# eukaryo/smith-waterman-simd

Measured on AMD Instinct MI355X. Metric: alignments/sec (and GCUPS) on 1M fixed-length pairs, 1/2/4/8 MI355X, higher is better.
Workload: dtype u16

## Files before the change

### smith-waterman-simd_amd/csrc/sw_kernels.hip

```cpp
#include "swmi_internal.h"

#include <type_traits>
#include <utility>

namespace swmi {
namespace {

constexpr int kSeqLen = 128;
constexpr int kWavesPerBlock = 4;


__device__ __forceinline__ int max_i16(int a, int b)
{
    const short r = __builtin_elementwise_max((short)a, (short)b);
    return (int)(unsigned short)r;
}

template <bool I16>
__device__ __forceinline__ int vmax(int a, int b)
{
    if constexpr (I16) return max_i16(a, b);
    else return a > b ? a : b;
}

template <bool I16>
__device__ __forceinline__ int sat_sub(int a, int b)
{
    if constexpr (I16) return (int)(unsigned short)__builtin_elementwise_sub_sat((unsigned short)a, (unsigned short)b);
    else return (int)__builtin_elementwise_sub_sat((unsigned)a, (unsigned)b);
}

__device__ __forceinline__ int keep(int v)
{
    asm volatile("" : "+v"(v));
    return v;
}

template <int L>
__device__ __forceinline__ int from_prev_lane(int v, int group_mask)
{
    if constexpr (L == 64) {
#ifdef SWMI_AB_SHFL_UP
        const int s = __shfl_up(v, 1);
        return (threadIdx.x & 63) ? s : 0;
#else
        return __builtin_amdgcn_update_dpp(0, v, 0x138 , 0xf, 0xf, true);
#endif
    } else if constexpr (L == 32) {
        return __builtin_amdgcn_update_dpp(0, v, 0x138, 0xf, 0xf, true) & group_mask;
    } else if constexpr (L == 16) {
        return __builtin_amdgcn_update_dpp(0, v, 0x111 , 0xf, 0xf, true);
    } else {
        return __builtin_amdgcn_update_dpp(0, v, 0x111, 0xf, 0xf, true) & group_mask;
    }
}

template <int R>
__device__ __forceinline__ void load_bases(const uint8_t *p, uint32_t (&w)[(R + 3) / 4])
{
    if constexpr (R == 2) {
        w[0] = *reinterpret_cast<const uint16_t *>(p);
    } else if constexpr (R == 4) {
        w[0] = *reinterpret_cast<const uint32_t *>(p);
    } else if constexpr (R == 8) {
        const uint2 v = *reinterpret_cast<const uint2 *>(p);
        w[0] = v.x; w[1] = v.y;
    } else {
#pragma unroll
        for (int k = 0; k < R / 16; ++k) {
            const uint4 v = *reinterpret_cast<const uint4 *>(p + 16 * k);
            w[4 * k + 0] = v.x; w[4 * k + 1] = v.y; w[4 * k + 2] = v.z; w[4 * k + 3] = v.w;
        }
    }
}

__device__ __forceinline__ uint32_t spread4(uint32_t v)
{
    return (v | (v << 6) | (v << 12) | (v << 18)) & 0x03030303u;
}

template <int R>
__device__ __forceinline__ void load_bases_packed(const uint8_t *p, uint32_t (&w)[(R + 3) / 4])
{
    if constexpr (R == 2) {
        w[0] = 0;
    } else if constexpr (R == 4) {
        w[0] = spread4(p[0]);
    } else if constexpr (R == 8) {
        const uint32_t v = *reinterpret_cast<const uint16_t *>(p);
        w[0] = spread4(v & 0xff); w[1] = spread4(v >> 8);
    } else if constexpr (R == 16) {
        const uint32_t v = *reinterpret_cast<const uint32_t *>(p);
#pragma unroll
        for (int k = 0; k < 4; ++k) w[k] = spread4((v >> (8 * k)) & 0xff);
    } else {
#pragma unroll
        for (int q = 0; q < R / 32; ++q) {
            const uint2 v = *reinterpret_cast<const uint2 *>(p + 8 * q);
#pragma unroll
            for (int k = 0; k < 4; ++k) {
                w[8 * q + k] = spread4((v.x >> (8 * k)) & 0xff);
                w[8 * q + 4 + k] = spread4((v.y >> (8 * k)) & 0xff);
            }
        }
    }
}

template <int L, bool FOLD, bool I16, int MODE>
__global__ void __launch_bounds__(64 * kWavesPerBlock)
sw128_kernel(const uint8_t *__restrict__ seq1s, const uint8_t *__restrict__ seq2s, int32_t *__restrict__ scores,
             uint32_t n, SmRows rows, int gap)
{
    constexpr int R = kSeqLen / L;
    constexpr int A = 64 / L;
    constexpr int PAD = L + 2;
    constexpr int S = kSeqLen + 2 * PAD;
    constexpr int T2 = (kSeqLen + L) / 2;
    constexpr int NW = (R + 3) / 4;

    constexpr bool kWideProfile = true;
    using profile_t = std::conditional_t<kWideProfile, uint32_t, uint16_t>;
    __shared__ profile_t lds_profile[kWavesPerBlock][A * S];
    __shared__ uint32_t lds_rows[kWavesPerBlock][4];
#ifndef SWMI_LDS_BEST_NUM
#define SWMI_LDS_BEST_NUM (R >= 64 ? 0 : R >= 32 ? 1 : R >= 16 ? 2 : R >= 8 ? 1 : 0)
#define SWMI_LDS_BEST_DEN (R >= 64 ? 1 : R >= 32 ? 2 : R >= 16 ? 3 : R >= 8 ? 2 : 1)
#endif
    constexpr int kBestNum = I16 ? 0 : SWMI_LDS_BEST_NUM, kBestDen = SWMI_LDS_BEST_DEN;
    __shared__ int lds_best[kWavesPerBlock][64];
    lds_best[threadIdx.x >> 6][threadIdx.x & 63] = 0;

    const int lane = threadIdx.x & 63;
    const int wv = threadIdx.x >> 6;
    const int g = lane / L;
    const int j = lane % L;
    const uint32_t first_pair = (blockIdx.x * kWavesPerBlock + wv) * A;
    if (first_pair >= n) return;
    uint32_t pair = first_pair + g;
    const bool live = pair < n;
    if (!live) pair = n - 1;

    uint32_t a_w[NW], b_w[NW];
    if constexpr (MODE == 1) {
        if constexpr (R == 2) {
            const uint32_t sh = 4 * (j & 1);
            a_w[0] = spread4((seq1s[(size_t)pair * 32 + (j >> 1)] >> sh) & 0xf);
            b_w[0] = spread4((seq2s[(size_t)pair * 32 + (j >> 1)] >> sh) & 0xf);
        } else {
            load_bases_packed<R>(seq1s + (size_t)pair * 32 + j * (R / 4), a_w);
            load_bases_packed<R>(seq2s + (size_t)pair * 32 + j * (R / 4), b_w);
        }
    } else {
        load_bases<R>(seq1s + (size_t)pair * kSeqLen + j * R, a_w);
        load_bases<R>(seq2s + (MODE == 2 ? (size_t)0 : (size_t)pair * kSeqLen) + j * R, b_w);
    }

    if (lane < 4) lds_rows[wv][lane] = rows.r[lane];
    profile_t *prof = &lds_profile[wv][g * S];
    for (int k = j; k < PAD; k += L) {
        prof[k] = 0;
        prof[PAD + kSeqLen + k] = 0;
    }
#pragma unroll
    for (int i = 0; i < R; ++i) {
        const uint32_t b = (b_w[i / 4] >> (8 * (i % 4))) & 3u;
        prof[PAD + j * R + i] = kWideProfile ? (profile_t)(1u << (8u * b)) : (profile_t)(0x100u | (8u * b));
    }
    __builtin_amdgcn_fence(__ATOMIC_RELEASE, "wavefront");
    __builtin_amdgcn_wave_barrier();
    __builtin_amdgcn_fence(__ATOMIC_ACQUIRE, "wavefront");

    int row_scores[R];
#pragma unroll
    for (int i = 0; i < R; ++i) {
        const uint32_t a = (a_w[i / 4] >> (8 * (i % 4))) & 3u;
        row_scores[i] = (int)lds_rows[wv][a];
    }

    __builtin_amdgcn_s_setprio(2);

    constexpr bool kKeepG = !FOLD && !I16;
    int h[R];
    int hg[kKeepG ? R : 1];
#pragma unroll
    for (int i = 0; i < R; ++i) h[i] = 0;
#pragma unroll
    for (int i = 0; i < (kKeepG ? R : 1); ++i) hg[i] = 0;
    int best = 0;
    int u0 = 0, u1 = 0;
    const int group_mask = keep(j == 0 ? 0 : -1);
    const profile_t *col = prof + PAD - j;

    auto step = [&](uint32_t entry, int up, int diag) {
        const int onehot = kWideProfile ? (int)entry : (int)((entry >> 8) << (entry & 31u));
        int dprev = diag;
        if constexpr (kKeepG) up = sat_sub<false>(up, gap);
#pragma unroll
        for (int i = 0; i < R; ++i) {
            const int left = h[i];
            const int tsum = __builtin_amdgcn_sdot4(row_scores[i], onehot, dprev, true);
            int hn;
            if constexpr (FOLD) {
                const int lu = left > up ? left : up;
                const int x = lu > tsum ? lu : tsum;
                if constexpr (I16) best = keep(max_i16(best, x));
                else if (i % kBestDen < kBestNum) __hip_atomic_fetch_max(&lds_best[wv][lane], x, __ATOMIC_RELAXED, __HIP_MEMORY_SCOPE_WAVEFRONT);
                else best = vmax<false>(best, x);
                hn = sat_sub<I16>(x, gap);
                up = hn;
            } else if constexpr (I16) {
                const int m = keep(max_i16(left, up));
                hn = keep(max_i16(sat_sub<true>(m, gap), tsum));
                best = keep(max_i16(best, hn));
                up = hn;
            } else {
                const int gl = hg[i];
                const int lu = gl > up ? gl : up;
                hn = lu > tsum ? lu : tsum;
                if (i % kBestDen < kBestNum) __hip_atomic_fetch_max(&lds_best[wv][lane], hn, __ATOMIC_RELAXED, __HIP_MEMORY_SCOPE_WAVEFRONT);
                else best = vmax<false>(best, hn);
                const int gn = sat_sub<false>(hn, gap);
                hg[i] = gn;
                up = gn;
            }
            h[i] = hn;
            dprev = left;
        }
        return from_prev_lane<L>(h[R - 1], group_mask);
    };

    uint32_t e0 = col[0];
    for (int t2 = 0; t2 < T2; ++t2) {
        const uint32_t e1 = col[2 * t2 + 1];
        const uint32_t e2 = col[2 * t2 + 2];
        u1 = step(e0, u0, u1);
        u0 = step(e1, u1, u0);
        e0 = e2;
    }

    if constexpr (kBestNum > 0) {
        const int from_lds = lds_best[wv][lane];
        best = best > from_lds ? best : from_lds;
    }
#pragma unroll
    for (int o = L / 2; o > 0; o >>= 1) {
        const int other = __shfl_xor(best, o);
        best = best > other ? best : other;
    }
    if constexpr (FOLD) best = best > gap ? best - gap : 0;
    if (j == 0 && live) scores[pair] = best;
}


__device__ __forceinline__ uint32_t pk_max3(uint32_t a, uint32_t b, uint32_t c)
{
    uint32_t r;
    asm("v_pk_maximum3_f16 %0, %1, %2, %3" : "=v"(r) : "v"(a), "v"(b), "v"(c));
    return r;
}
__device__ __forceinline__ void keep_f16_denormals()
{
    asm volatile("s_setreg_imm32_b32 hwreg(HW_REG_MODE, 6, 2), 3");
}

constexpr uint32_t kPkLimit = 0x7C00u;
constexpr uint32_t kBPerThread = 1024;
__global__ void __launch_bounds__(256)
pk_max3_selftest_kernel(unsigned long long *__restrict__ counts )
{
    keep_f16_denormals();
    const uint32_t a = blockIdx.x * 256 + threadIdx.x;
    const uint32_t b0 = blockIdx.y * kBPerThread;
    if (a >= kPkLimit) return;
    auto imax3 = [](uint32_t p, uint32_t q, uint32_t r) { const uint32_t m = p > q ? p : q; return m > r ? m : r; };
    auto pk_max3 = [](uint32_t p, uint32_t q, uint32_t r) {
        uint32_t o;
        asm volatile("v_pk_maximum3_f16 %0, %1, %2, %3\n\ts_nop 1" : "=v"(o) : "v"(p), "v"(q), "v"(r));
        return o;
    };
    uint32_t bad = 0, done = 0;
    for (uint32_t b = b0; b < b0 + kBPerThread && b < kPkLimit; ++b) {
        uint32_t h = (a * 0x9E3779B1u) ^ (b * 0x85EBCA77u);
        h ^= h >> 15; h *= 0x2C1B3C6Du; h ^= h >> 12;
        const uint32_t r = h % kPkLimit, r2 = (h >> 7) % kPkLimit;
        const uint32_t x = a | (b << 16), y = b | (r << 16), z = r2 | (a << 16);
        bad += pk_max3(x, y, z) != (imax3(a, b, r2) | (imax3(b, r, a) << 16));
        bad += pk_max3(z, x, y) != (imax3(r2, a, b) | (imax3(a, b, r) << 16));
        bad += pk_max3(y, z, x) != (imax3(b, r2, a) | (imax3(r, a, b) << 16));
        bad += pk_max3(x, y, x) != (imax3(a, b, a) | (imax3(b, r, b) << 16));
        bad += pk_max3(x, y, y) != (imax3(a, b, b) | (imax3(b, r, r) << 16));
        bad += pk_max3(x, x, y) != (imax3(a, a, b) | (imax3(b, b, r) << 16));
        done += 6;
    }
    atomicAdd(&counts[0], (unsigned long long)done);
    if (bad) atomicAdd(&counts[1], (unsigned long long)bad);
}
template <bool LAST>
__device__ __forceinline__ void pk_two_rows(uint32_t &hq0, uint32_t &hq1, uint32_t &hu0, uint32_t &hu1, uint32_t &best, uint32_t &t,
                                            uint32_t &sc, uint32_t up, uint32_t sel2, uint32_t sel3, uint32_t cx, uint32_t cy,
                                            uint32_t gq2, uint32_t q2)
{
    uint32_t x0, x1, s2;
    if constexpr (!LAST) {
        asm volatile("v_pk_maximum3_f16 %[x0], %[hq0], %[up], %[t]\n\t"
                     "v_add_u32 %[t], %[hu0], %[sc]\n\t"
                     "s_nop 0\n\t"
                     "v_pk_sub_u16 %[hu0], %[x0], %[gq] clamp\n\t"
                     "v_perm_b32 %[s2], %[cy], %[cx], %[sel2]\n\t"
                     "v_add_u32 %[hq0], %[q], %[hu0]\n\t"
                     "s_nop 0\n\t"
                     "v_pk_maximum3_f16 %[x1], %[hq1], %[hq0], %[t]\n\t"
                     "v_add_u32 %[t], %[hu1], %[s2]\n\t"
                     "s_nop 0\n\t"
                     "v_pk_sub_u16 %[hu1], %[x1], %[gq] clamp\n\t"
                     "v_perm_b32 %[sc], %[cy], %[cx], %[sel3]\n\t"
                     "s_nop 0\n\t"
                     "v_add_u32 %[hq1], %[q], %[hu1]\n\t"
                     "v_pk_maximum3_f16 %[best], %[best], %[x0], %[x1]"
                     : [hq0] "+v"(hq0), [hq1] "+v"(hq1), [hu0] "+v"(hu0), [hu1] "+v"(hu1), [best] "+v"(best), [t] "+v"(t),
                       [sc] "+v"(sc), [x0] "=&v"(x0), [x1] "=&v"(x1), [s2] "=&v"(s2)
                     : [up] "v"(up), [sel2] "v"(sel2), [sel3] "v"(sel3), [cx] "v"(cx), [cy] "v"(cy), [gq] "s"(gq2), [q] "s"(q2));
    } else {
        asm volatile("v_pk_maximum3_f16 %[x0], %[hq0], %[up], %[t]\n\t"
                     "v_add_u32 %[t], %[hu0], %[sc]\n\t"
                     "s_nop 0\n\t"
                     "v_pk_sub_u16 %[hu0], %[x0], %[gq] clamp\n\t"
                     "s_nop 0\n\t"
                     "v_add_u32 %[hq0], %[q], %[hu0]\n\t"
                     "s_nop 0\n\t"
                     "v_pk_maximum3_f16 %[x1], %[hq1], %[hq0], %[t]\n\t"
                     "s_nop 0\n\t"
                     "v_pk_sub_u16 %[hu1], %[x1], %[gq] clamp\n\t"
                     "v_pk_maximum3_f16 %[best], %[best], %[x0], %[x1]\n\t"
                     "v_add_u32 %[hq1], %[q], %[hu1]"
                     : [hq0] "+v"(hq0), [hq1] "+v"(hq1), [hu0] "+v"(hu0), [hu1] "+v"(hu1), [best] "+v"(best), [t] "+v"(t),
                       [x0] "=&v"(x0), [x1] "=&v"(x1)
                     : [up] "v"(up), [sc] "v"(sc), [gq] "s"(gq2), [q] "s"(q2));
    }
}

enum PkVariant : int { kPkQ0 = 0, kPkBias = 1, kPkVert = 2 };
constexpr int kPkProductBit = 1 << 16;

template <int MODE, int VARIANT, int L>
__global__ void __launch_bounds__(64 * kWavesPerBlock) __attribute__((amdgpu_waves_per_eu(4)))
sw128_pk_kernel(const uint8_t *__restrict__ seq1s, const uint8_t *__restrict__ seq2s, int32_t *__restrict__ scores,
                uint32_t n, SmRows rows ,
                int gap, int q_arg )
{
    const int q = VARIANT == kPkVert ? q_arg & (kPkProductBit - 1) : q_arg;
    const bool product = VARIANT == kPkVert && (q_arg & kPkProductBit) != 0;
    static_assert(L == 4 || L == 8 || L == 16, "lanes per pair of alignments");
    constexpr bool kGenerated = VARIANT == kPkQ0 || VARIANT == kPkVert;
    constexpr int R = kSeqLen / L;
    constexpr int G = 64 / L;
    constexpr int A = 2 * G;
    constexpr int PAD = L + 2;
    constexpr int S = kSeqLen + 2 * PAD;
    constexpr int T2 = (kSeqLen + L - 1) / 2;
    constexpr int NW = R / 4;
    constexpr uint32_t kPadCode = 16u | (16u << 16);
    const bool flag_form = VARIANT == kPkVert && q != 0;

    __shared__ uint32_t lds_col[kWavesPerBlock][G * S];
    __shared__ uint32_t lds_tab[8];

    const int lane = threadIdx.x & 63;
    const int wv = threadIdx.x >> 6;
    const int g = lane / L, j = lane % L;
    const uint32_t first = (blockIdx.x * kWavesPerBlock + wv) * A;
    if (first >= n) return;
    uint32_t px = first + 2 * g, py = px + 1;
    const bool live_x = px < n, live_y = py < n;
    if (!live_x) px = n - 1;
    if (!live_y) py = n - 1;

    uint32_t ax[NW], bx[NW], ay[NW], by[NW];
    if constexpr (MODE == 1) {
        load_bases_packed<R>(seq1s + (size_t)px * 32 + j * (R / 4), ax);
        load_bases_packed<R>(seq2s + (size_t)px * 32 + j * (R / 4), bx);
        load_bases_packed<R>(seq1s + (size_t)py * 32 + j * (R / 4), ay);
        load_bases_packed<R>(seq2s + (size_t)py * 32 + j * (R / 4), by);
    } else {
        load_bases<R>(seq1s + (size_t)px * kSeqLen + j * R, ax);
        load_bases<R>(seq2s + (MODE == 2 ? (size_t)0 : (size_t)px * kSeqLen) + j * R, bx);
        load_bases<R>(seq1s + (size_t)py * kSeqLen + j * R, ay);
        load_bases<R>(seq2s + (MODE == 2 ? (size_t)0 : (size_t)py * kSeqLen) + j * R, by);
    }

    if (lane < 5) {
        uint32_t c = flag_form ? 0x80808080u : 0u;
        if (lane < 4) {
            c = 0;
#pragma unroll
            for (int a = 0; a < 4; ++a) c |= ((rows.r[a] >> (8 * lane)) & 0xFFu) << (8 * a);
        }
        lds_tab[lane] = c;
    }
    uint32_t *prof = &lds_col[wv][g * S];
    const uint32_t pad_code = product ? 0u : kPadCode;
    for (int k = j; k < PAD; k += L) {
        prof[k] = pad_code;
        prof[PAD + kSeqLen + k] = pad_code;
    }
    const uint32_t sel_shift = flag_form ? 8u : 0u, sel_const = flag_form ? 0x000D000Du : 0x0C000C00u;
    uint32_t rsel[R];
    if (product) {
#pragma unroll
        for (int w = 0; w < NW; ++w) {
            const uint32_t cx4 = bx[w] & 0x03030303u, cy4 = by[w] & 0x03030303u;
            const uint32_t ra4 = ax[w] & 0x03030303u, rb4 = ay[w] & 0x03030303u;
#pragma unroll
            for (int k = 0; k < 4; ++k) {
                const uint32_t pick = (uint32_t)k | 0x0C000C00u | ((uint32_t)(4 + k) << 16);
                const uint32_t ce = __builtin_amdgcn_perm(cy4, cx4, pick), re = __builtin_amdgcn_perm(rb4, ra4, pick);
                prof[PAD + j * R + 4 * w + k] = __builtin_amdgcn_perm(rows.r[3], rows.r[2], ((ce * 0x101u) << 1) + 0x01000100u);
                rsel[4 * w + k] = __builtin_amdgcn_perm(rows.r[1], rows.r[0], ((re * 0x101u) << 1) + 0x01000100u);
            }
        }
    } else {
#pragma unroll
    for (int w = 0; w < NW; ++w) {
        const uint32_t cx4 = (bx[w] & 0x03030303u) << 2, cy4 = (by[w] & 0x03030303u) << 2;
        const uint32_t ra4 = ax[w] & 0x03030303u, rb4 = (ay[w] & 0x03030303u) | 0x04040404u;
#pragma unroll
        for (int k = 0; k < 4; ++k) {
            const uint32_t pick = (uint32_t)k | 0x0C000C00u | ((uint32_t)(4 + k) << 16);
            prof[PAD + j * R + 4 * w + k] = __builtin_amdgcn_perm(cy4, cx4, pick);
            if constexpr (VARIANT == kPkVert) rsel[4 * w + k] = (__builtin_amdgcn_perm(rb4, ra4, pick) << sel_shift) | sel_const;
            else                              rsel[4 * w + k] = __builtin_amdgcn_perm(rb4, ra4, pick) | 0x0C000C00u;
        }
    }
    }
    __builtin_amdgcn_fence(__ATOMIC_RELEASE, "wavefront");
    __builtin_amdgcn_wave_barrier();
    __builtin_amdgcn_fence(__ATOMIC_ACQUIRE, "wavefront");
    __builtin_amdgcn_s_setprio(2);

    keep_f16_denormals();

    const uint32_t gq2 = (uint32_t)(gap + q) | ((uint32_t)(gap + q) << 16);
    const uint32_t q2 = (uint32_t)q | ((uint32_t)q << 16);
    uint32_t best = 0;
    const int group_mask = keep(j == 0 ? 0 : -1);
    const uint32_t *col = prof + PAD - j;
    auto tables = [&](uint32_t code, uint32_t &cx, uint32_t &cy) {
        cx = *reinterpret_cast<const uint32_t *>(reinterpret_cast<const char *>(lds_tab) + (code & 0xFFFFu));
        cy = *reinterpret_cast<const uint32_t *>(reinterpret_cast<const char *>(lds_tab) + (code >> 16));
    };
    auto tables_at = [&](int t, uint32_t &cx, uint32_t &cy) {
        const uint16_t *half = reinterpret_cast<const uint16_t *>(col + t);
        cx = *reinterpret_cast<const uint32_t *>(reinterpret_cast<const char *>(lds_tab) + half[0]);
        cy = *reinterpret_cast<const uint32_t *>(reinterpret_cast<const char *>(lds_tab) + half[1]);
    };

    if constexpr (kGenerated) {
#define pk_best best
#define pk_dval(r) ((uint32_t)(gap * ((r) + 1)) * 0x10001u)
        if constexpr (VARIANT == kPkQ0 && R == 32) {
#define PK_SECTION 32
#include "pk_sweeps_gen.inc"
#undef PK_SECTION
        } else if constexpr (VARIANT == kPkQ0 && R == 16) {
#define PK_SECTION 16
#include "pk_sweeps_gen.inc"
#undef PK_SECTION
        } else if constexpr (VARIANT == kPkQ0 && R == 8) {
#define PK_SECTION 8
#include "pk_sweeps_gen.inc"
#undef PK_SECTION
        } else if (product) {
            if constexpr (R == 32) {
#define PK_SECTION 432
#include "pk_sweeps_gen.inc"
#undef PK_SECTION
            } else if constexpr (R == 16) {
#define PK_SECTION 416
#include "pk_sweeps_gen.inc"
#undef PK_SECTION
            } else {
#define PK_SECTION 408
#include "pk_sweeps_gen.inc"
#undef PK_SECTION
            }
        } else if (flag_form) {
            if constexpr (R == 32) {
#define PK_SECTION 332
#include "pk_sweeps_gen.inc"
#undef PK_SECTION
            } else if constexpr (R == 16) {
#define PK_SECTION 316
#include "pk_sweeps_gen.inc"
#undef PK_SECTION
            } else {
#define PK_SECTION 308
#include "pk_sweeps_gen.inc"
#undef PK_SECTION
            }
        } else if constexpr (VARIANT == kPkVert && R == 32) {
#define PK_SECTION 232
#include "pk_sweeps_gen.inc"
#undef PK_SECTION
        } else if constexpr (VARIANT == kPkVert && R == 16) {
#define PK_SECTION 216
#include "pk_sweeps_gen.inc"
#undef PK_SECTION
        } else {
#define PK_SECTION 208
#include "pk_sweeps_gen.inc"
#undef PK_SECTION
        }
#undef pk_best
#undef pk_dval
    } else {
    uint32_t hq[R], hu_[R];
#pragma unroll
    for (int i = 0; i < R; ++i) { hq[i] = q2; hu_[i] = 0; }
    uint32_t u0 = q2, u1 = q2;
    const uint32_t edge = (uint32_t)keep((int)(j == 0 ? q2 : 0u));

    auto step = [&](uint32_t cx, uint32_t cy, uint32_t up, uint32_t diag) {
        const uint32_t d0 = diag - q2;
        uint32_t t = d0 + __builtin_amdgcn_perm(cy, cx, rsel[0]);
        uint32_t sc = __builtin_amdgcn_perm(cy, cx, rsel[1]);
#pragma unroll
        for (int i = 0; i < R; i += 2) {
            if (i + 2 < R) pk_two_rows<false>(hq[i], hq[i + 1], hu_[i], hu_[i + 1], best, t, sc, up, rsel[i + 2], rsel[i + 3], cx, cy, gq2, q2);
            else           pk_two_rows<true>(hq[i], hq[i + 1], hu_[i], hu_[i + 1], best, t, sc, up, 0, 0, cx, cy, gq2, q2);
            up = hq[i + 1];
        }
        asm volatile("s_nop 1");
        uint32_t out = (uint32_t)from_prev_lane<L>((int)hq[R - 1], group_mask);
        return out | edge;
    };
    uint32_t c1 = col[1], x0, y0;
    tables(col[0], x0, y0);
    for (int t2 = 0; t2 < T2; ++t2) {
        const uint32_t c2 = col[2 * t2 + 2], c3 = col[2 * t2 + 3];
        uint32_t x1, y1, x2, y2;
        tables(c1, x1, y1);
        u1 = step(x0, y0, u0, u1);
        tables(c2, x2, y2);
        u0 = step(x1, y1, u1, u0);
        x0 = x2; y0 = y2; c1 = c3;
    }
    step(x0, y0, u0, u1);
    }

#pragma unroll
    for (int o = L / 2; o > 0; o >>= 1) {
        const uint32_t other = (uint32_t)__shfl_xor((int)best, o);
        best = pk_max3(best, other, other);
    }
    const int bx_score = (int)(best & 0xFFFFu), by_score = (int)(best >> 16), gq = VARIANT != kPkVert ? gap + q : flag_form ? gap : 0;
    int sx = bx_score > gq ? bx_score - gq : 0, sy = by_score > gq ? by_score - gq : 0;
    if (flag_form) {
        sx = sx * q / 255;
        sy = sy * q / 255;
    }
    if (j == 0) {
        if (live_x) scores[px] = sx;
        if (live_y) scores[py] = sy;
    }
}

template <int ROW>
__device__ __forceinline__ void fetch_score(int &dst, uint32_t lds_addr)
{
    asm volatile("ds_read_i8 %0, %1 offset:%2" : "=v"(dst) : "v"(lds_addr), "i"(ROW * 256));
}
template <int R, int... I>
__device__ __forceinline__ void fetch_scores_impl(int (&dst)[R], uint32_t lds_addr, std::integer_sequence<int, I...>)
{
    (fetch_score<I>(dst[I], lds_addr), ...);
}
template <int R>
__device__ __forceinline__ void fetch_scores(int (&dst)[R], uint32_t lds_addr)
{
    fetch_scores_impl<R>(dst, lds_addr, std::make_integer_sequence<int, R>{});
}
template <int R>
__device__ __forceinline__ void land_scores(int (&s)[R])
{
    asm volatile("s_waitcnt lgkmcnt(0)" ::: "memory");
#pragma unroll
    for (int i = 0; i < R; ++i) asm volatile("" : "+v"(s[i]));
}

template <int L, int MODE>
__global__ void __launch_bounds__(64 * kWavesPerBlock)
sw128_lut_kernel(const uint8_t *__restrict__ seq1s, const uint8_t *__restrict__ seq2s, int32_t *__restrict__ scores,
                 uint32_t n, SmRows rows, int gap)
{
    constexpr int R = kSeqLen / L;
    constexpr int A = 64 / L;
    constexpr int PAD = L + 4;
    constexpr int S = kSeqLen + 2 * PAD;
    constexpr int T2 = (kSeqLen + L - 1 + 1) / 2;
    constexpr int NW = (R + 3) / 4;

    __shared__ int lds_colofs[kWavesPerBlock][A * S];
    __shared__ uint32_t lds_q[kWavesPerBlock][R * 64];
    __shared__ uint32_t lds_neg[R * 64];
    __shared__ uint32_t lds_rows[kWavesPerBlock][4];

    for (int k = threadIdx.x; k < R * 64; k += 64 * kWavesPerBlock) lds_neg[k] = 0x80808080u;
    __syncthreads();

    const int lane = threadIdx.x & 63;
    const int wv = threadIdx.x >> 6;
    const int g = lane / L;
    const int j = lane % L;
    const uint32_t first_pair = (blockIdx.x * kWavesPerBlock + wv) * A;
    if (first_pair >= n) return;
    uint32_t pair = first_pair + g;
    const bool live = pair < n;
    if (!live) pair = n - 1;

    uint32_t a_w[NW], b_w[NW];
    if constexpr (MODE == 1) {
        if constexpr (R == 2) {
            const uint32_t sh = 4 * (j & 1);
            a_w[0] = spread4((seq1s[(size_t)pair * 32 + (j >> 1)] >> sh) & 0xf);
            b_w[0] = spread4((seq2s[(size_t)pair * 32 + (j >> 1)] >> sh) & 0xf);
        } else {
            load_bases_packed<R>(seq1s + (size_t)pair * 32 + j * (R / 4), a_w);
            load_bases_packed<R>(seq2s + (size_t)pair * 32 + j * (R / 4), b_w);
        }
    } else {
        load_bases<R>(seq1s + (size_t)pair * kSeqLen + j * R, a_w);
        load_bases<R>(seq2s + (MODE == 2 ? (size_t)0 : (size_t)pair * kSeqLen) + j * R, b_w);
    }

    if (lane < 4) lds_rows[wv][lane] = rows.r[lane];
    const int neg_ofs = (int)((const char *)lds_neg - (const char *)lds_q[wv]);
    int *prof = &lds_colofs[wv][g * S];
    for (int k = j; k < PAD; k += L) {
        prof[k] = neg_ofs;
        prof[PAD + kSeqLen + k] = neg_ofs;
    }
#pragma unroll
    for (int i = 0; i < R; ++i) prof[PAD + j * R + i] = (int)((b_w[i / 4] >> (8 * (i % 4))) & 3u);
    __builtin_amdgcn_fence(__ATOMIC_RELEASE, "wavefront");
    __builtin_amdgcn_wave_barrier();
    __builtin_amdgcn_fence(__ATOMIC_ACQUIRE, "wavefront");
#pragma unroll
    for (int i = 0; i < R; ++i) {
        const uint32_t a = (a_w[i / 4] >> (8 * (i % 4))) & 3u;
        lds_q[wv][i * 64 + lane] = lds_rows[wv][a];
    }
    __builtin_amdgcn_fence(__ATOMIC_RELEASE, "wavefront");
    __builtin_amdgcn_wave_barrier();
    __builtin_amdgcn_fence(__ATOMIC_ACQUIRE, "wavefront");

    const uint32_t qlane = (uint32_t)(uintptr_t)(&lds_q[wv][lane]);
    const int *col = prof + PAD - j;

    int h[R];
#pragma unroll
    for (int i = 0; i < R; ++i) h[i] = 0;
    int best = 0;
    int u0 = 0, u1 = 0;
    const int group_mask = keep(j == 0 ? 0 : -1);

    int sA[R], sB[R];
    fetch_scores<R>(sA, qlane + (uint32_t)col[0]);
    int ofs_next = col[1];

    auto step = [&](const int (&sc)[R], int up, int diag) {
        int dprev = diag;
#pragma unroll
        for (int i = 0; i < R; ++i) {
            const int left = h[i];
            const int tsum = dprev + sc[i];
            const int lu = left > up ? left : up;
            const int x = lu > tsum ? lu : tsum;
            best = best > x ? best : x;
            const int hn = sat_sub<false>(x, gap);
            h[i] = hn;
            up = hn;
            dprev = left;
        }
        return from_prev_lane<L>(up, group_mask);
    };

    for (int t2 = 0; t2 < T2; ++t2) {
        {
            land_scores<R>(sA);
            fetch_scores<R>(sB, qlane + (uint32_t)ofs_next);
            ofs_next = col[2 * t2 + 2];
            u1 = step(sA, u0, u1);
        }
        {
            land_scores<R>(sB);
            fetch_scores<R>(sA, qlane + (uint32_t)ofs_next);
            ofs_next = col[2 * t2 + 3];
            u0 = step(sB, u1, u0);
        }
    }
    land_scores<R>(sA);

#pragma unroll
    for (int o = L / 2; o > 0; o >>= 1) {
        const int other = __shfl_xor(best, o);
        best = best > other ? best : other;
    }
    best = best > gap ? best - gap : 0;
    if (j == 0 && live) scores[pair] = best;
}

__device__ __forceinline__ int below_minus(int v, int ext)
{
    return __builtin_amdgcn_update_dpp(0, v, 0x138 , 0xf, 0xf, true) - ext;
}
__device__ __forceinline__ int above_minus(int v, int ext)
{
    return __builtin_amdgcn_update_dpp(0, v, 0x130 , 0xf, 0xf, true) - ext;
}

#ifndef SWMI_BA_NOPS
#define SWMI_BA_NOPS 9
#endif
#define BA_NOP(bit, v) do { if constexpr ((SWMI_BA_NOPS >> (bit)) & 1) asm volatile("s_nop 0" : "+v"(v)); } while (0)
template <bool kOpenGeExt, bool kI16>
__global__ void __launch_bounds__(64 * kWavesPerBlock)
sw_banded_affine_kernel(const uint8_t *__restrict__ seq1s, const uint8_t *__restrict__ seq2s, int32_t *__restrict__ scores,
                        uint32_t n, int len, SmRows rows, int gap_open, int gap_ext)
{
    extern __shared__ uint32_t lds_dyn[];
    __shared__ uint32_t lds_rows[kWavesPerBlock][4];
    const int lane = threadIdx.x & 63;
    const int wv = threadIdx.x >> 6;
    const uint32_t pair = blockIdx.x * kWavesPerBlock + wv;
    if (pair >= n) return;
    const int stride = len + 72;
    uint32_t *arow = lds_dyn + (size_t)wv * 2 * stride;
    uint32_t *boh = arow + stride;

    if (lane < 4) lds_rows[wv][lane] = rows.r[lane];
    __builtin_amdgcn_fence(__ATOMIC_RELEASE, "wavefront");
    __builtin_amdgcn_wave_barrier();
    __builtin_amdgcn_fence(__ATOMIC_ACQUIRE, "wavefront");
    const uint8_t *s1 = seq1s + (size_t)pair * (size_t)len;
    const uint8_t *s2 = seq2s + (size_t)pair * (size_t)len;
    for (int kp = lane; kp < stride; kp += 64) {
        const int k = kp - 32;
        const bool in = (unsigned)k < (unsigned)len;
        const uint32_t a = in ? (s1[k] & 3u) : 0u;
        const uint32_t b = in ? (s2[k] & 3u) : 0u;
        arow[kp] = in ? lds_rows[wv][a] : 0x80808080u;
        boh[kp] = in ? (1u << (8u * b)) : 0u;
    }
    __builtin_amdgcn_fence(__ATOMIC_RELEASE, "wavefront");
    __builtin_amdgcn_wave_barrier();
    __builtin_amdgcn_fence(__ATOMIC_ACQUIRE, "wavefront");

    const uint32_t *pa = arow + (64 - lane);
    const uint32_t *pb = boh + lane;
    int a_cur = (int)pa[0];
    int b_cur = (int)pb[0];
    int best = 0;

    {
        const int step_cost = kOpenGeExt ? gap_ext : gap_open;
        const int fold = kOpenGeExt ? gap_open - gap_ext : gap_ext - gap_open;
        const int cost_v = keep(step_cost);
        int h0 = 0, me0 = 0, mf0 = 0;
        int h1 = 0, me1 = 0, mf1 = 0;
        auto hand_over = [&](int h, int e, int f, int &me, int &mf) {
            if constexpr (kOpenGeExt) {
                int hm = sat_sub<false>(h, fold);
                BA_NOP(1, hm);
                me = vmax<kI16>(e, hm);
                BA_NOP(2, me);
                mf = vmax<kI16>(f, hm);
                BA_NOP(3, mf);
            } else {
                const int em = e - fold, fm = f - fold;
                me = vmax<kI16>(em, h);
                mf = vmax<kI16>(fm, h);
                BA_NOP(3, mf);
            }
        };
        auto pair_of_steps = [&](int b_next) {
            {
                const int e = below_minus(me1, cost_v);
                int f = sat_sub<false>(mf1, step_cost);
                BA_NOP(0, f);
                const int t = __builtin_amdgcn_sdot4(a_cur, b_cur, h0, true);
                const int tf = t > f ? t : f;
                h0 = tf > e ? tf : e;
                hand_over(h0, e, f, me0, mf0);
            }
            b_cur = b_next;
            {
                int e = sat_sub<false>(me0, step_cost);
                BA_NOP(0, e);
                const int f = above_minus(mf0, cost_v);
                const int t = __builtin_amdgcn_sdot4(a_cur, b_cur, h1, true);
                const int te = t > e ? t : e;
                h1 = te > f ? te : f;
                hand_over(h1, e, f, me1, mf1);
            }
            const int hb = h0 > h1 ? h0 : h1;
            best = best > hb ? best : hb;
        };
        int u = 0;
#pragma unroll 1
        for (; u + 4 <= len; u += 4) {
            const int b1 = (int)pb[u + 1], b2 = (int)pb[u + 2], b3 = (int)pb[u + 3], b4 = (int)pb[u + 4];
            const int a1 = (int)pa[u + 1], a2 = (int)pa[u + 2], a3 = (int)pa[u + 3], a4 = (int)pa[u + 4];
            pair_of_steps(b1); a_cur = a1;
            pair_of_steps(b2); a_cur = a2;
            pair_of_steps(b3); a_cur = a3;
            pair_of_steps(b4); a_cur = a4;
        }
        for (; u < len; ++u) {
            const int b_next = (int)pb[u + 1];
            const int a_next = (int)pa[u + 1];
            pair_of_steps(b_next);
            a_cur = a_next;
        }
    }
#pragma unroll
    for (int o = 32; o > 0; o >>= 1) {
        const int other = __shfl_xor(best, o);
        best = best > other ? best : other;
    }
    if (lane == 0) scores[pair] = best;
}

__device__ __forceinline__ unsigned ba_pk_max3(unsigned a, unsigned b, unsigned c)
{
    typedef _Float16 h2 __attribute__((ext_vector_type(2)));
    const h2 m = __builtin_elementwise_maximum(__builtin_elementwise_maximum(__builtin_bit_cast(h2, a), __builtin_bit_cast(h2, b)), __builtin_bit_cast(h2, c));
    return __builtin_bit_cast(unsigned, m);
}
__device__ __forceinline__ unsigned ba_pk_sub_sat(unsigned v, unsigned d)
{
    typedef unsigned short us2 __attribute__((ext_vector_type(2)));
    return __builtin_bit_cast(unsigned, __builtin_elementwise_sub_sat(__builtin_bit_cast(us2, v), __builtin_bit_cast(us2, d)));
}

struct BandedPkParams {
    uint32_t rows[4];
    uint32_t bias2;
    uint32_t fold2;
    uint32_t cost2;
    uint32_t delta2;
    uint32_t best_step;
};

constexpr int kBandedTrip = 16;
template <bool kOpenGeExt>
__global__ void __launch_bounds__(64 * kWavesPerBlock)
sw_banded_affine_pk_kernel(const uint8_t *__restrict__ seq1s, const uint8_t *__restrict__ seq2s, int32_t *__restrict__ scores,
                           uint32_t n, int len, BandedPkParams prm)
{
    extern __shared__ uint32_t lds_dyn[];
    __shared__ uint32_t lds_rows[kWavesPerBlock][4];
    const int lane = threadIdx.x & 63;
    const int wv = threadIdx.x >> 6;
    const uint32_t wave_id = blockIdx.x * kWavesPerBlock + wv;
    const uint32_t pair_x = 2 * wave_id;
    if (pair_x >= n) return;
    const uint32_t pair_y = pair_x + 1 < n ? pair_x + 1 : pair_x;
    const int stride = len + 72;
    uint2 *arow = reinterpret_cast<uint2 *>(lds_dyn + (size_t)wv * 3 * stride);
    uint32_t *bsel = lds_dyn + (size_t)wv * 3 * stride + 2 * stride;

    keep_f16_denormals();
    if (lane < 4) lds_rows[wv][lane] = prm.rows[lane];
    __builtin_amdgcn_fence(__ATOMIC_RELEASE, "wavefront");
    __builtin_amdgcn_wave_barrier();
    __builtin_amdgcn_fence(__ATOMIC_ACQUIRE, "wavefront");
    const uint8_t *x1 = seq1s + (size_t)pair_x * (size_t)len, *x2 = seq2s + (size_t)pair_x * (size_t)len;
    const uint8_t *y1 = seq1s + (size_t)pair_y * (size_t)len, *y2 = seq2s + (size_t)pair_y * (size_t)len;
    for (int kp = lane; kp < stride; kp += 64) {
        const int k = kp - 32;
        const bool in = (unsigned)k < (unsigned)len;
        const uint32_t ax = in ? (x1[k] & 3u) : 0u, ay = in ? (y1[k] & 3u) : 0u;
        const uint32_t bx = in ? (x2[k] & 3u) : 0u, by = in ? (y2[k] & 3u) : 0u;
        arow[kp] = in ? make_uint2(lds_rows[wv][ax], lds_rows[wv][ay]) : make_uint2(0u, 0u);
        bsel[kp] = in ? (0x0C000C00u | bx | ((4u + by) << 16)) : 0x0C0C0C0Cu;
    }
    __builtin_amdgcn_fence(__ATOMIC_RELEASE, "wavefront");
    __builtin_amdgcn_wave_barrier();
    __builtin_amdgcn_fence(__ATOMIC_ACQUIRE, "wavefront");

    const uint2 *pa = arow + (64 - lane);
    const uint32_t *pb = bsel + lane;
    uint2 a_cur = pa[0];
    uint32_t b_cur = pb[0];
    const unsigned bias2 = prm.bias2, fold2 = prm.fold2, cost2 = prm.cost2;
    const unsigned delta_left = lane == 0 ? 0u : prm.delta2, cost_up = lane == 63 ? 0u : cost2;
    const unsigned long long own_step = (unsigned long long)prm.delta2 | ((unsigned long long)prm.best_step << 32);
    unsigned best = 0;
    unsigned h0 = 0, h1 = 0;
    unsigned me0 = cost2, mf0 = cost2, me1 = cost2, mf1 = cost2;
    auto hand_over = [&](unsigned m, unsigned e, unsigned f, unsigned floor2, unsigned &me, unsigned &mf) {
        if constexpr (kOpenGeExt) {
            const unsigned hm = ba_pk_sub_sat(m, fold2);
            me = ba_pk_max3(e, hm, floor2);
            mf = ba_pk_max3(f, hm, floor2);
        } else {
            const unsigned em = ba_pk_sub_sat(e, fold2), fm = ba_pk_sub_sat(f, fold2);
            me = ba_pk_max3(em, m, floor2);
            mf = ba_pk_max3(fm, m, floor2);
        }
    };
    auto pair_of_steps = [&](uint32_t b_next, unsigned floor2) {
        const unsigned p0 = __builtin_amdgcn_perm(a_cur.y, a_cur.x, b_cur), p1 = __builtin_amdgcn_perm(a_cur.y, a_cur.x, b_next);
        unsigned long long t, fb;
        asm("v_lshl_add_u64 %0, %1, 0, %2" : "=v"(t) : "v"((unsigned long long)h0 | ((unsigned long long)h1 << 32)),
                                                        "v"((unsigned long long)p0 | ((unsigned long long)p1 << 32)));
        const unsigned t0 = (unsigned)t, t1 = (unsigned)(t >> 32);
        {
            const unsigned e = (unsigned)__builtin_amdgcn_update_dpp(0, (int)me1, 0x138 , 0xf, 0xf, true) + delta_left;
            asm("v_lshl_add_u64 %0, %1, 0, %2" : "=v"(fb) : "v"((unsigned long long)mf1 | ((unsigned long long)best << 32)), "s"(own_step));
            const unsigned f = (unsigned)fb;
            best = (unsigned)(fb >> 32);
            h0 = ba_pk_max3(t0, e, f);
            hand_over(h0, e, f, floor2, me0, mf0);
        }
        {
            const unsigned e = me0 - cost2;
            const unsigned f = (unsigned)__builtin_amdgcn_update_dpp(0, (int)mf0, 0x130 , 0xf, 0xf, true) - cost_up;
            h1 = ba_pk_max3(t1, e, f);
            hand_over(h1, e, f, floor2, me1, mf1);
        }
        best = ba_pk_max3(best, h0, h1);
        b_cur = b_next;
    };
    auto rebase = [&](unsigned back2) {
        h0 -= back2; h1 -= back2; me0 -= back2; mf0 -= back2; me1 -= back2; mf1 -= back2; best -= back2;
    };
    int u = 0;
#pragma unroll 1
    for (; u + kBandedTrip <= len; u += kBandedTrip) {
#pragma unroll
        for (int k = 0; k < kBandedTrip; ++k) {
            const uint32_t b_next = pb[u + k + 1];
            const uint2 a_next = pa[u + k + 1];
            pair_of_steps(b_next, cost2 + (unsigned)(k + 1) * bias2);
            a_cur = a_next;
        }
        rebase((unsigned)kBandedTrip * bias2);
    }
    for (; u < len; ++u) {
        const uint32_t b_next = pb[u + 1];
        const uint2 a_next = pa[u + 1];
        pair_of_steps(b_next, cost2 + bias2);
        a_cur = a_next;
        rebase(bias2);
    }
    int bx = (int)(best & 0xFFFFu), by = (int)(best >> 16);
#pragma unroll
    for (int o = 32; o > 0; o >>= 1) {
        const int ox = __shfl_xor(bx, o), oy = __shfl_xor(by, o);
        bx = bx > ox ? bx : ox;
        by = by > oy ? by : oy;
    }
    if (lane == 0) {
        scores[pair_x] = bx;
        if (pair_x + 1 < n) scores[pair_x + 1] = by;
    }
}


__device__ __forceinline__ uint64_t splitmix64(uint64_t z)
{
    z += 0x9E3779B97F4A7C15ull;
    z = (z ^ (z >> 30)) * 0xBF58476D1CE4E5B9ull;
    z = (z ^ (z >> 27)) * 0x94D049BB133111EBull;
    return z ^ (z >> 31);
}

__global__ void __launch_bounds__(256)
generate_kernel(uint8_t *__restrict__ seq1s, uint8_t *__restrict__ seq2s, uint64_t n_words, uint64_t seed,
                uint64_t first_pair)
{
    const uint64_t stride = (uint64_t)gridDim.x * blockDim.x;
    for (uint64_t id = (uint64_t)blockIdx.x * blockDim.x + threadIdx.x; id < n_words; id += stride) {
        const uint64_t w = id & 3, s = (id >> 2) & 1, k = id >> 3;
        const uint64_t ctr = ((first_pair + k) * 2 + s) * 4 + w;
        const uint64_t x = splitmix64(seed ^ (ctr * 0x9E3779B97F4A7C15ull));
        uint4 lo, hi;
        lo.x = spread4((uint32_t)(x >> 0) & 0xff);  lo.y = spread4((uint32_t)(x >> 8) & 0xff);
        lo.z = spread4((uint32_t)(x >> 16) & 0xff); lo.w = spread4((uint32_t)(x >> 24) & 0xff);
        hi.x = spread4((uint32_t)(x >> 32) & 0xff); hi.y = spread4((uint32_t)(x >> 40) & 0xff);
        hi.z = spread4((uint32_t)(x >> 48) & 0xff); hi.w = spread4((uint32_t)(x >> 56) & 0xff);
        uint4 *dst = reinterpret_cast<uint4 *>((s ? seq2s : seq1s) + k * kSeqLen + w * 32);
        dst[0] = lo;
        dst[1] = hi;
    }
}

__global__ void __launch_bounds__(256)
unpack_kernel(const uint8_t *__restrict__ packed, uint8_t *__restrict__ unpacked, uint64_t n_words)
{
    const uint64_t stride = (uint64_t)gridDim.x * blockDim.x;
    for (uint64_t id = (uint64_t)blockIdx.x * blockDim.x + threadIdx.x; id < n_words; id += stride) {
        const uint32_t v = reinterpret_cast<const uint32_t *>(packed)[id];
        uint4 o;
        o.x = spread4(v & 0xff); o.y = spread4((v >> 8) & 0xff);
        o.z = spread4((v >> 16) & 0xff); o.w = spread4(v >> 24);
        reinterpret_cast<uint4 *>(unpacked)[id] = o;
    }
}

template <int L, int MODE>
hipError_t launch_L(const LaunchConfig &cfg, const uint8_t *s1, const uint8_t *s2, int32_t *out, size_t n,
                    const SmRows &rows, int gap, hipStream_t stream)
{
    constexpr int A = 64 / L;
    const size_t waves = (n + A - 1) / A;
    const size_t blocks = (waves + kWavesPerBlock - 1) / kWavesPerBlock;
    if (blocks == 0) return hipSuccess;
    if (blocks > 0x7fffffffull || n > 0xffffffffull) return hipErrorInvalidValue;
    const dim3 grid((unsigned)blocks), block(64 * kWavesPerBlock);
    const uint32_t n32 = (uint32_t)n;
    if constexpr (L == 4 || L == 8 || L == 16) {
        if (cfg.use_pk) {
            const size_t waves_pk = (n + 2 * A - 1) / (2 * A);
            const dim3 grid_pk((unsigned)((waves_pk + kWavesPerBlock - 1) / kWavesPerBlock));
            switch (cfg.pk_variant) {
            case kPkQ0:    hipLaunchKernelGGL((sw128_pk_kernel<MODE, kPkQ0, L>), grid_pk, block, cfg.extra_lds_bytes, stream, s1, s2, out, n32, rows, gap, 0); break;
            case kPkVert:  hipLaunchKernelGGL((sw128_pk_kernel<MODE, kPkVert, L>), grid_pk, block, cfg.extra_lds_bytes, stream, s1, s2, out, n32, rows,
                                              cfg.pk_flag_unit ? cfg.pk_flag_gap : gap, cfg.pk_flag_unit | (cfg.pk_product ? kPkProductBit : 0)); break;
            default:       hipLaunchKernelGGL((sw128_pk_kernel<MODE, kPkBias, L>), grid_pk, block, cfg.extra_lds_bytes, stream, s1, s2, out, n32, rows, gap, cfg.pk_bias); break;
            }
            return hipGetLastError();
        }
    }
    if constexpr (L <= 16 && L >= 4) {
        if (cfg.fold_gap && cfg.use_lut) {
            hipLaunchKernelGGL((sw128_lut_kernel<L, MODE>), grid, block, cfg.extra_lds_bytes, stream, s1, s2, out, n32, rows, gap);
            return hipGetLastError();
        }
    }
    if (cfg.fold_gap) {
        if (cfg.use_i16) hipLaunchKernelGGL((sw128_kernel<L, true, true, MODE>), grid, block, cfg.extra_lds_bytes, stream, s1, s2, out, n32, rows, gap);
        else             hipLaunchKernelGGL((sw128_kernel<L, true, false, MODE>), grid, block, cfg.extra_lds_bytes, stream, s1, s2, out, n32, rows, gap);
    } else {
        if (cfg.use_i16) hipLaunchKernelGGL((sw128_kernel<L, false, true, MODE>), grid, block, cfg.extra_lds_bytes, stream, s1, s2, out, n32, rows, gap);
        else             hipLaunchKernelGGL((sw128_kernel<L, false, false, MODE>), grid, block, cfg.extra_lds_bytes, stream, s1, s2, out, n32, rows, gap);
    }
    return hipGetLastError();
}

template <int MODE>
hipError_t launch_mode(const LaunchConfig &cfg, const uint8_t *s1, const uint8_t *s2, int32_t *out, size_t n,
                       const SmRows &rows, int gap, hipStream_t stream)
{
    switch (cfg.lanes_per_alignment) {
    case 64: return launch_L<64, MODE>(cfg, s1, s2, out, n, rows, gap, stream);
    case 32: return launch_L<32, MODE>(cfg, s1, s2, out, n, rows, gap, stream);
    case 16: return launch_L<16, MODE>(cfg, s1, s2, out, n, rows, gap, stream);
    case 8:  return launch_L<8, MODE>(cfg, s1, s2, out, n, rows, gap, stream);
    case 4:  return launch_L<4, MODE>(cfg, s1, s2, out, n, rows, gap, stream);
    case 2:  return launch_L<2, MODE>(cfg, s1, s2, out, n, rows, gap, stream);
    default: return hipErrorInvalidValue;
    }
}

}

bool schedule_supported(int L)
{
    return L == 64 || L == 32 || L == 16 || L == 8 || L == 4 || L == 2;
}

hipError_t launch_score(const LaunchConfig &cfg, const uint8_t *d_seq1s, const uint8_t *d_seq2s, int32_t *d_scores,
                        size_t n, const SmRows &rows, int gap, bool packed, hipStream_t stream)
{
    return packed ? launch_mode<1>(cfg, d_seq1s, d_seq2s, d_scores, n, rows, gap, stream)
                  : launch_mode<0>(cfg, d_seq1s, d_seq2s, d_scores, n, rows, gap, stream);
}

hipError_t launch_score_one_vs_many(const LaunchConfig &cfg, const uint8_t *d_seq1s, const uint8_t *d_seq2,
                                    int32_t *d_scores, size_t n_seq1, const SmRows &rows, int gap, hipStream_t stream)
{
    return launch_mode<2>(cfg, d_seq1s, d_seq2, d_scores, n_seq1, rows, gap, stream);
}

int banded_affine_kernel_choice(int len, const SmRows &rows, int gap_open, int gap_ext, bool allow_i16, bool allow_pk)
{
    int top = 0, low = 0;
    for (int a = 0; a < 4; ++a)
        for (int b = 0; b < 4; ++b) {
            const int v = (int)(int8_t)(rows.r[a] >> (8 * b));
            top = v > top ? v : top;
            low = v < low ? v : low;
        }
    const long long bias = -low;
    if (allow_pk && (long long)len * top + (kBandedTrip + 2) * bias + gap_open + gap_ext + 64 < 0x7C00) return 2;
    return (long long)len * top < 32768 && allow_i16 ? 1 : 0;
}

hipError_t launch_banded_affine(const uint8_t *d_seq1s, const uint8_t *d_seq2s, int32_t *d_scores, size_t n, int len,
                                const SmRows &rows, int gap_open, int gap_ext, hipStream_t stream, bool allow_i16, bool allow_pk)
{
    if (n == 0) return hipSuccess;
    const int choice = banded_affine_kernel_choice(len, rows, gap_open, gap_ext, allow_i16, allow_pk);
    const dim3 block(64 * kWavesPerBlock);
    if (choice == 2) {
        const size_t waves = (n + 1) / 2, blocks = (waves + kWavesPerBlock - 1) / kWavesPerBlock;
        if (blocks > 0x7fffffffull) return hipErrorInvalidValue;
        const size_t lds = (size_t)kWavesPerBlock * 3 * (size_t)(len + 72) * sizeof(uint32_t);
        int low = 0;
        for (int a = 0; a < 4; ++a)
            for (int b = 0; b < 4; ++b) {
                const int v = (int)(int8_t)(rows.r[a] >> (8 * b));
                low = v < low ? v : low;
            }
        const unsigned bias = (unsigned)-low;
        BandedPkParams prm;
        for (int a = 0; a < 4; ++a) {
            uint32_t r = 0;
            for (int b = 0; b < 4; ++b) r |= (uint32_t)((int)(int8_t)(rows.r[a] >> (8 * b)) + (int)bias) << (8 * b);
            prm.rows[a] = r;
        }
        const bool oge = gap_open >= gap_ext;
        const unsigned fold = (unsigned)(oge ? gap_open - gap_ext : gap_ext - gap_open), cost = (unsigned)(oge ? gap_ext : gap_open);
        prm.bias2 = bias * 0x10001u;
        prm.fold2 = fold * 0x10001u;
        prm.cost2 = cost * 0x10001u;
        if (bias >= cost) {
            prm.delta2 = (bias - cost) * 0x10001u;
            prm.best_step = prm.bias2;
        } else {
            const unsigned d = cost - bias;
            prm.delta2 = ((0x10000u - d) & 0xFFFFu) | (((0x10000u - d - 1u) & 0xFFFFu) << 16);
            prm.best_step = prm.bias2 - 1u;
        }
        const dim3 grid((unsigned)blocks);
        if (oge) hipLaunchKernelGGL((sw_banded_affine_pk_kernel<true>), grid, block, lds, stream, d_seq1s, d_seq2s, d_scores, (uint32_t)n, len, prm);
        else     hipLaunchKernelGGL((sw_banded_affine_pk_kernel<false>), grid, block, lds, stream, d_seq1s, d_seq2s, d_scores, (uint32_t)n, len, prm);
        return hipGetLastError();
    }
    const size_t blocks = (n + kWavesPerBlock - 1) / kWavesPerBlock;
    if (blocks > 0x7fffffffull) return hipErrorInvalidValue;
    const size_t lds = (size_t)kWavesPerBlock * 2 * (size_t)(len + 72) * sizeof(uint32_t);
    const bool i16 = choice == 1;
    const dim3 grid((unsigned)blocks);
    if (gap_open >= gap_ext) {
        if (i16) hipLaunchKernelGGL((sw_banded_affine_kernel<true, true>), grid, block, lds, stream, d_seq1s, d_seq2s, d_scores, (uint32_t)n, len, rows, gap_open, gap_ext);
        else     hipLaunchKernelGGL((sw_banded_affine_kernel<true, false>), grid, block, lds, stream, d_seq1s, d_seq2s, d_scores, (uint32_t)n, len, rows, gap_open, gap_ext);
    } else {
        if (i16) hipLaunchKernelGGL((sw_banded_affine_kernel<false, true>), grid, block, lds, stream, d_seq1s, d_seq2s, d_scores, (uint32_t)n, len, rows, gap_open, gap_ext);
        else     hipLaunchKernelGGL((sw_banded_affine_kernel<false, false>), grid, block, lds, stream, d_seq1s, d_seq2s, d_scores, (uint32_t)n, len, rows, gap_open, gap_ext);
    }
    return hipGetLastError();
}

hipError_t launch_pk_max3_selftest(unsigned long long *d_counts, hipStream_t stream)
{
    const dim3 grid((kPkLimit + 255) / 256, (kPkLimit + kBPerThread - 1) / kBPerThread);
    hipLaunchKernelGGL(pk_max3_selftest_kernel, grid, dim3(256), 0, stream, d_counts);
    return hipGetLastError();
}

hipError_t launch_generate(uint8_t *d_seq1s, uint8_t *d_seq2s, size_t n, uint64_t seed, uint64_t first_pair,
                           hipStream_t stream)
{
    if (n == 0) return hipSuccess;
    const uint64_t n_words = (uint64_t)n * 8;
    uint64_t blocks = (n_words + 255) / 256;
    if (blocks > 65536) blocks = 65536;
    hipLaunchKernelGGL(generate_kernel, dim3((unsigned)blocks), dim3(256), 0, stream, d_seq1s, d_seq2s, n_words, seed,
                       first_pair);
    return hipGetLastError();
}

hipError_t launch_unpack(const uint8_t *d_packed, uint8_t *d_unpacked, size_t n_seqs, hipStream_t stream)
{
    if (n_seqs == 0) return hipSuccess;
    const uint64_t n_words = (uint64_t)n_seqs * 8;
    uint64_t blocks = (n_words + 255) / 256;
    if (blocks > 65536) blocks = 65536;
    hipLaunchKernelGGL(unpack_kernel, dim3((unsigned)blocks), dim3(256), 0, stream, d_packed, d_unpacked, n_words);
    return hipGetLastError();
}

}
```

Measured before the change: 1.250 billion.

## Store banded pk sequence rows as byte indices into shared lookup tables

The banded packed-u16 kernel now keeps one byte per position in LDS: an index into a 16-entry shared table of substitution row pairs and selector words, replacing the previous 12 bytes per position. Preprocessing reads sequences with 16-byte vector loads when aligned, and the inner loop software-pipelines the index fetch and table lookup two steps ahead. This cuts LDS footprint (more waves per CU) and global load instructions, at the cost of an extra dependent LDS lookup per step.

```diff
diff --git a/smith-waterman-simd_amd/csrc/sw_kernels.hip b/smith-waterman-simd_amd/csrc/sw_kernels.hip
--- a/smith-waterman-simd_amd/csrc/sw_kernels.hip
+++ b/smith-waterman-simd_amd/csrc/sw_kernels.hip
@@ -852,46 +852,69 @@
 };
 
 constexpr int kBandedTrip = 16;
+constexpr uint32_t kBandedPadRow = 16u * 8u, kBandedPadSel = 16u * 4u;
+__host__ __device__ constexpr int banded_pk_stride(int len) { return (len + 72 + 15) & ~15; }
+__device__ __forceinline__ uint32_t ba_pk_index4(uint32_t x, uint32_t y, int shift)
+{
+    return (((x & 0x03030303u) << 2) | (y & 0x03030303u)) << shift;
+}
 template <bool kOpenGeExt>
 __global__ void __launch_bounds__(64 * kWavesPerBlock)
 sw_banded_affine_pk_kernel(const uint8_t *__restrict__ seq1s, const uint8_t *__restrict__ seq2s, int32_t *__restrict__ scores,
                            uint32_t n, int len, BandedPkParams prm)
 {
     extern __shared__ uint32_t lds_dyn[];
-    __shared__ uint32_t lds_rows[kWavesPerBlock][4];
+    __shared__ uint2 tab_rows[17];
+    __shared__ uint32_t tab_sel[17];
     const int lane = threadIdx.x & 63;
     const int wv = threadIdx.x >> 6;
     const uint32_t wave_id = blockIdx.x * kWavesPerBlock + wv;
     const uint32_t pair_x = 2 * wave_id;
     if (pair_x >= n) return;
     const uint32_t pair_y = pair_x + 1 < n ? pair_x + 1 : pair_x;
-    const int stride = len + 72;
-    uint2 *arow = reinterpret_cast<uint2 *>(lds_dyn + (size_t)wv * 3 * stride);
-    uint32_t *bsel = lds_dyn + (size_t)wv * 3 * stride + 2 * stride;
+    const int stride = banded_pk_stride(len);
+    uint32_t *arow4 = lds_dyn + (size_t)wv * 2 * (stride / 4), *bsel4 = arow4 + stride / 4;
+    uint8_t *arow = reinterpret_cast<uint8_t *>(arow4), *bsel = reinterpret_cast<uint8_t *>(bsel4);
 
     keep_f16_denormals();
-    if (lane < 4) lds_rows[wv][lane] = prm.rows[lane];
+    if (lane < 17) {
+        const uint32_t hi = (uint32_t)lane >> 2, lo = (uint32_t)lane & 3u;
+        auto row_of = [&](uint32_t a) { return a == 0 ? prm.rows[0] : a == 1 ? prm.rows[1] : a == 2 ? prm.rows[2] : prm.rows[3]; };
+        tab_rows[lane] = lane < 16 ? make_uint2(row_of(hi), row_of(lo)) : make_uint2(0u, 0u);
+        tab_sel[lane] = lane < 16 ? (0x0C000C00u | hi | ((4u + lo) << 16)) : 0x0C0C0C0Cu;
+    }
+    const uint8_t *x1 = seq1s + (size_t)pair_x * (size_t)len, *x2 = seq2s + (size_t)pair_x * (size_t)len;
+    const uint8_t *y1 = seq1s + (size_t)pair_y * (size_t)len, *y2 = seq2s + (size_t)pair_y * (size_t)len;
+    if (lane < 32) { arow[lane] = (uint8_t)kBandedPadRow; bsel[lane] = (uint8_t)kBandedPadSel; }
+    for (int kp = len + 32 + lane; kp < stride; kp += 64) { arow[kp] = (uint8_t)kBandedPadRow; bsel[kp] = (uint8_t)kBandedPadSel; }
+    if ((((uintptr_t)seq1s | (uintptr_t)seq2s | (uintptr_t)(unsigned)len) & 15u) == 0) {
+        for (int c = lane; c < (len >> 4); c += 64) {
+            const uint4 vx1 = reinterpret_cast<const uint4 *>(x1)[c], vy1 = reinterpret_cast<const uint4 *>(y1)[c];
+            const uint4 vx2 = reinterpret_cast<const uint4 *>(x2)[c], vy2 = reinterpret_cast<const uint4 *>(y2)[c];
+            uint32_t *wa = arow4 + 8 + 4 * c, *wb = bsel4 + 8 + 4 * c;
+            wa[0] = ba_pk_index4(vx1.x, vy1.x, 3); wa[1] = ba_pk_index4(vx1.y, vy1.y, 3);
+            wa[2] = ba_pk_index4(vx1.z, vy1.z, 3); wa[3] = ba_pk_index4(vx1.w, vy1.w, 3);
+            wb[0] = ba_pk_index4(vx2.x, vy2.x, 2); wb[1] = ba_pk_index4(vx2.y, vy2.y, 2);
+            wb[2] = ba_pk_index4(vx2.z, vy2.z, 2); wb[3] = ba_pk_index4(vx2.w, vy2.w, 2);
+        }
+    } else {
+        for (int k = lane; k < len; k += 64) {
+            const uint32_t ax = x1[k] & 3u, ay = y1[k] & 3u, bx = x2[k] & 3u, by = y2[k] & 3u;
+            arow[32 + k] = (uint8_t)((ax << 2 | ay) << 3);
+            bsel[32 + k] = (uint8_t)((bx << 2 | by) << 2);
+        }
+    }
     __builtin_amdgcn_fence(__ATOMIC_RELEASE, "wavefront");
     __builtin_amdgcn_wave_barrier();
     __builtin_amdgcn_fence(__ATOMIC_ACQUIRE, "wavefront");
-    const uint8_t *x1 = seq1s + (size_t)pair_x * (size_t)len, *x2 = seq2s + (size_t)pair_x * (size_t)len;
-    const uint8_t *y1 = seq1s + (size_t)pair_y * (size_t)len, *y2 = seq2s + (size_t)pair_y * (size_t)len;
-    for (int kp = lane; kp < stride; kp += 64) {
-        const int k = kp - 32;
-        const bool in = (unsigned)k < (unsigned)len;
-        const uint32_t ax = in ? (x1[k] & 3u) : 0u, ay = in ? (y1[k] & 3u) : 0u;
-        const uint32_t bx = in ? (x2[k] & 3u) : 0u, by = in ? (y2[k] & 3u) : 0u;
-        arow[kp] = in ? make_uint2(lds_rows[wv][ax], lds_rows[wv][ay]) : make_uint2(0u, 0u);
-        bsel[kp] = in ? (0x0C000C00u | bx | ((4u + by) << 16)) : 0x0C0C0C0Cu;
-    }
-    __builtin_amdgcn_fence(__ATOMIC_RELEASE, "wavefront");
-    __builtin_amdgcn_wave_barrier();
-    __builtin_amdgcn_fence(__ATOMIC_ACQUIRE, "wavefront");
-
-    const uint2 *pa = arow + (64 - lane);
-    const uint32_t *pb = bsel + lane;
-    uint2 a_cur = pa[0];
-    uint32_t b_cur = pb[0];
+
+    const uint8_t *pa = arow + (64 - lane);
+    const uint8_t *pb = bsel + lane;
+    auto rows_at = [&](uint32_t off) { return *reinterpret_cast<const uint2 *>(reinterpret_cast<const uint8_t *>(tab_rows) + off); };
+    auto sel_at = [&](uint32_t off) { return *reinterpret_cast<const uint32_t *>(reinterpret_cast<const uint8_t *>(tab_sel) + off); };
+    uint2 a_cur = rows_at(pa[0]);
+    uint32_t b_cur = sel_at(pb[0]), b_nx1 = sel_at(pb[1]);
+    uint32_t ia_nx1 = pa[1], ib_nx2 = pb[2];
     const unsigned bias2 = prm.bias2, fold2 = prm.fold2, cost2 = prm.cost2;
     const unsigned delta_left = lane == 0 ? 0u : prm.delta2, cost_up = lane == 63 ? 0u : cost2;
     const unsigned long long own_step = (unsigned long long)prm.delta2 | ((unsigned long long)prm.best_step << 32);
@@ -940,18 +963,24 @@
     for (; u + kBandedTrip <= len; u += kBandedTrip) {
 #pragma unroll
         for (int k = 0; k < kBandedTrip; ++k) {
-            const uint32_t b_next = pb[u + k + 1];
-            const uint2 a_next = pa[u + k + 1];
-            pair_of_steps(b_next, cost2 + (unsigned)(k + 1) * bias2);
-            a_cur = a_next;
+            const uint2 a_nx1 = rows_at(ia_nx1);
+            const uint32_t b_nx2 = sel_at(ib_nx2);
+            ia_nx1 = pa[u + k + 2];
+            ib_nx2 = pb[u + k + 3];
+            pair_of_steps(b_nx1, cost2 + (unsigned)(k + 1) * bias2);
+            a_cur = a_nx1;
+            b_nx1 = b_nx2;
         }
         rebase((unsigned)kBandedTrip * bias2);
     }
     for (; u < len; ++u) {
-        const uint32_t b_next = pb[u + 1];
-        const uint2 a_next = pa[u + 1];
-        pair_of_steps(b_next, cost2 + bias2);
-        a_cur = a_next;
+        const uint2 a_nx1 = rows_at(ia_nx1);
+        const uint32_t b_nx2 = sel_at(ib_nx2);
+        ia_nx1 = pa[u + 2];
+        ib_nx2 = pb[u + 3];
+        pair_of_steps(b_nx1, cost2 + bias2);
+        a_cur = a_nx1;
+        b_nx1 = b_nx2;
         rebase(bias2);
     }
     int bx = (int)(best & 0xFFFFu), by = (int)(best >> 16);
@@ -1107,7 +1136,7 @@
     if (choice == 2) {
         const size_t waves = (n + 1) / 2, blocks = (waves + kWavesPerBlock - 1) / kWavesPerBlock;
         if (blocks > 0x7fffffffull) return hipErrorInvalidValue;
-        const size_t lds = (size_t)kWavesPerBlock * 3 * (size_t)(len + 72) * sizeof(uint32_t);
+        const size_t lds = (size_t)kWavesPerBlock * 2 * (size_t)banded_pk_stride(len);
         int low = 0;
         for (int a = 0; a < 4; ++a)
             for (int b = 0; b < 4; ++b) {
```

Result: no change. 1.249 billion (-0.1%).
